# yzqin/s4g-release

Hardware: AMD Instinct MI355X
Metric: scenes/sec (25.6k-pt clouds) end-to-end grasp inference (higher is better)
Workload: dtype f32 (f16x2 split)

## Files before the change

### s4g_release_amd/csrc/fps.hip

```cpp
#include <stdlib.h>
#include <string.h>


#include "s4g_common.h"

namespace s4g {

constexpr int FPS_THREADS = 1024;
constexpr int FPS_TIE_PAR = 5;
constexpr int FPS_MAX_WAVES = 16;
constexpr uint32_t FPS_JMASK = 0x7FFFFFu;

typedef float fps_v2f __attribute__((ext_vector_type(2)));

struct FpsSlot {
  uint32_t d;
  uint32_t tie;
  float x, y, z;
  uint32_t d2;
  uint32_t key2;
  uint32_t pad;
};

struct FpsExtra {
// ... 144 lines not shown
        wkey = min(wkey, dpp_u32<0x141>(wkey));
        const bool was_hit = v != s.d;
        uint32_t kb = (was_hit && s.d2 == bnd) ? slots[ej].key2 : 0xFFFFFFFFu;
        kb = min(kb, dpp_u32<0xB1>(kb));
        kb = min(kb, dpp_u32<0x4E>(kb));
        kb = min(kb, dpp_u32<0x141>(kb));
        if (!((uint32_t)__builtin_amdgcn_readlane(wkey, 0) < (uint32_t)__builtin_amdgcn_readlane(kb, 0))) break;
      }
      take(k);
    }
  }
  cur = (int)((uint32_t)__builtin_amdgcn_readlane(s.tie, xl) & FPS_JMASK);
  cx = __uint_as_float(__builtin_amdgcn_readlane(__float_as_uint(s.x), xl));
  cy = __uint_as_float(__builtin_amdgcn_readlane(__float_as_uint(s.y), xl));
  cz = __uint_as_float(__builtin_amdgcn_readlane(__float_as_uint(s.z), xl));
  fx = __uint_as_float(__builtin_amdgcn_readlane(__float_as_uint(s.x), xl0));
  fy = __uint_as_float(__builtin_amdgcn_readlane(__float_as_uint(s.y), xl0));
  fz = __uint_as_float(__builtin_amdgcn_readlane(__float_as_uint(s.z), xl0));
  if (wave == 0 && lane < np) {
    const FpsSlot e = slots[(pw >> (4 * lane)) & 15u];
    out_i[lane] = (IdxT)(e.tie & FPS_JMASK);
    if (cout_i) {
      cout_i[lane] = e.x;
      cout_i[M + lane] = e.y;
      cout_i[2 * M + lane] = e.z;
    }
    if (dout_i) dout_i[lane] = __uint_as_float(my_d);
  }
  picked_waves = pw;
  return np;
}

template <int PPT, int LO, int HI>
__device__ __forceinline__ void fps_pick(const float (&x)[PPT],
                                         const float (&y)[PPT],
                                         const float (&z)[PPT], int pw, int wl,
                                         float& sx, float& sy, float& sz) {
  if constexpr (HI - LO == 1) {
    sx = __uint_as_float(__builtin_amdgcn_readlane(__float_as_uint(x[LO]), wl));
    sy = __uint_as_float(__builtin_amdgcn_readlane(__float_as_uint(y[LO]), wl));
    sz = __uint_as_float(__builtin_amdgcn_readlane(__float_as_uint(z[LO]), wl));
  } else {
    constexpr int MID = (LO + HI) / 2;
    if (pw < MID)
      fps_pick<PPT, LO, MID>(x, y, z, pw, wl, sx, sy, sz);
    else
      fps_pick<PPT, MID, HI>(x, y, z, pw, wl, sx, sy, sz);
  }
}

template <int THREADS, int PPT, bool FMAD, typename IdxT>
__global__ __launch_bounds__(THREADS) void fps_reg_kernel(
    const float* __restrict__ xyz, int N, int M, IdxT* __restrict__ idx,
    float* __restrict__ ctr, int lg_bs, int M_run, float* __restrict__ md_out, FpsExtra ex) {
  constexpr int WAVES = THREADS / 64;
  __shared__ FpsSlot slots[2][FPS_MAX_WAVES];
  const int b = blockIdx.x;
  const int t = threadIdx.x;
  const int lane = t & 63;
  const int wave = t >> 6;
  const float* __restrict__ px = xyz + (size_t)b * 3 * N;
  const float* __restrict__ py = px + N;
  const float* __restrict__ pz = py + N;
  IdxT* __restrict__ out = idx + (size_t)b * M;
  float* __restrict__ cout = ctr ? ctr + (size_t)b * 3 * M : nullptr;
  float* __restrict__ dout = ex.dist ? ex.dist + (size_t)b * M : nullptr;
  if (ex.run && ex.run[b] == 0) {
    for (int i = t; i < M_run; i += THREADS) {
      out[i] = (IdxT)i;
      if (cout) {
        cout[i] = px[i];
        cout[M + i] = py[i];
        cout[2 * M + i] = pz[i];
      }
    }
    return;
  }

  float x[PPT], y[PPT], z[PPT], md[PPT];
#pragma unroll
  for (int p = 0; p < PPT; ++p) {
    const int j = t + THREADS * p;
    const bool ok = j < N;
    const int jj = ok ? j : 0;
    x[p] = px[jj];
    y[p] = py[jj];
    z[p] = pz[jj];
    md[p] = ok ? __builtin_inff() : -1.0f;
  }
  const uint32_t bs_mask = (1u << lg_bs) - 1u;
  const uint32_t rkey = (__brev((uint32_t)t & bs_mask) >> (32 - lg_bs)) << 23;

  int cur = 0;
  float cx = px[0], cy = py[0], cz = pz[0];
  if (t == 0) {
    out[0] = 0;
    if (cout) {
      cout[0] = cx;
      cout[M] = cy;
      cout[2 * M] = cz;
    }
    if (dout) dout[0] = __builtin_inff();
  }

  for (int i = 1; i < M_run; ++i) {
    float best = 0.0f;
    int bestp = -1;
    const fps_v2f cx2 = {cx, cx}, cy2 = {cy, cy}, cz2 = {cz, cz};
#pragma unroll
    for (int p = 0; p + 1 < PPT; p += 2) {
      const fps_v2f xv = {x[p], x[p + 1]}, yv = {y[p], y[p + 1]}, zv = {z[p], z[p + 1]};
      const fps_v2f dx = xv - cx2, dy = yv - cy2, dz = zv - cz2;
      fps_v2f d;
      if constexpr (FMAD) {
        d = __builtin_elementwise_fma(dz, dz, __builtin_elementwise_fma(dy, dy, dx * dx));
      } else {
        d = (dx * dx + dy * dy) + dz * dz;
      }
#pragma unroll
      for (int e = 0; e < 2; ++e) {
        float m;
        asm("v_min_f32 %0, %1, %2" : "=v"(m) : "v"(d[e]), "v"(md[p + e]));
        md[p + e] = m;
        if (m > best) {
          best = m;
          bestp = p + e;
        }
      }
    }
    if constexpr (PPT & 1) {
      constexpr int p = PPT - 1;
      const float d = dist2<FMAD>(cx, cy, cz, x[p], y[p], z[p]);
      float m;
      asm("v_min_f32 %0, %1, %2" : "=v"(m) : "v"(d), "v"(md[p]));
      md[p] = m;
      if (m > best) {
        best = m;
        bestp = p;
      }
    }
    const uint32_t jbest =
        (bestp < 0) ? (uint32_t)cur : (uint32_t)(t + THREADS * bestp);
    const uint32_t tie = rkey | jbest;
    const uint32_t dbits = __float_as_uint(best);
    const uint32_t wmax = wave_max_u32(dbits);
    uint64_t win = __ballot(dbits == wmax);
    uint32_t wtie;
    if (__popcll(win) > 1) {
      wtie = wave_min_u32((dbits == wmax) ? tie : 0xFFFFFFFFu);
      win = __ballot(dbits == wmax && tie == wtie);
    } else {
      wtie = __builtin_amdgcn_readlane(tie, __ffsll((unsigned long long)win) - 1);
    }
    const int wl = __ffsll((unsigned long long)win) - 1;
    const int pw = __builtin_amdgcn_readlane(bestp, wl);
    float sx = cx, sy = cy, sz = cz;
    if (pw >= 0) fps_pick<PPT, 0, PPT>(x, y, z, pw, wl, sx, sy, sz);
    uint32_t dwin;
    fps_block_exchange<WAVES>(slots[i & 1], wave, lane, wmax, wtie, sx, sy, sz, cur,
                       cx, cy, cz, &dwin);
    if (t == 0) {
      out[i] = (IdxT)cur;
      if (cout) {
        cout[i] = cx;
        cout[M + i] = cy;
        cout[2 * M + i] = cz;
      }
      if (dout) dout[i] = __uint_as_float(dwin);
    }
  }
  if (md_out) {
#pragma unroll
    for (int p = 0; p < PPT; ++p) {
      const int j = t + THREADS * p;
      if (j < N) md_out[(size_t)b * N + j] = md[p];
    }
  }
}

template <bool FMAD, typename IdxT>
__global__ __launch_bounds__(FPS_THREADS) void fps_stream_kernel(
    const float* __restrict__ xyz, int N, int M, IdxT* __restrict__ idx,
    float* __restrict__ ctr, float* __restrict__ temp, int lg_bs) {
  __shared__ FpsSlot slots[2][FPS_MAX_WAVES];
  const int b = blockIdx.x;
  const int t = threadIdx.x;
  const int lane = t & 63;
  const int wave = t >> 6;
  const float* __restrict__ px = xyz + (size_t)b * 3 * N;
  const float* __restrict__ py = px + N;
  const float* __restrict__ pz = py + N;
  float* __restrict__ md = temp + (size_t)b * N;
  IdxT* __restrict__ out = idx + (size_t)b * M;
  float* __restrict__ cout = ctr ? ctr + (size_t)b * 3 * M : nullptr;

  for (int j = t; j < N; j += FPS_THREADS) md[j] = __builtin_inff();
  const uint32_t bs_mask = (1u << lg_bs) - 1u;
  const uint32_t rkey = (__brev((uint32_t)t & bs_mask) >> (32 - lg_bs)) << 23;

  int cur = 0;
  float cx = px[0], cy = py[0], cz = pz[0];
  if (t == 0) {
    out[0] = 0;
    if (cout) {
      cout[0] = cx;
      cout[M] = cy;
      cout[2 * M] = cz;
    }
  }

  for (int i = 1; i < M; ++i) {
    float best = 0.0f;
    int bestj = -1;
    for (int j = t; j < N; j += FPS_THREADS) {
      const float d = dist2<FMAD>(cx, cy, cz, px[j], py[j], pz[j]);
      const float o = md[j];
      const float m = (d < o) ? d : o;
      if (d < o) md[j] = m;
      if (m > best) {
        best = m;
        bestj = j;
      }
    }
    const uint32_t jbest = (bestj < 0) ? (uint32_t)cur : (uint32_t)bestj;
    const uint32_t tie = rkey | jbest;
    const uint32_t dbits = __float_as_uint(best);
    const uint32_t wmax = wave_max_u32(dbits);
    const uint32_t wtie = wave_min_u32((dbits == wmax) ? tie : 0xFFFFFFFFu);
// ... 361 lines not shown
      for (int u = 0; u < AU; ++u) {
        const int sp = sp0 + u * FPS_SORT_THREADS;
        j[u] = sp < N ? __hip_atomic_load(&pm[sp], __ATOMIC_RELAXED, __HIP_MEMORY_SCOPE_AGENT) : 0;
      }
      float c[AU][3];
#pragma unroll
      for (int u = 0; u < AU; ++u)
#pragma unroll
        for (int a = 0; a < 3; ++a) c[u][a] = p[(size_t)a * N + j[u]];
#pragma unroll
      for (int u = 0; u < AU; ++u) {
        const int sp = sp0 + u * FPS_SORT_THREADS;
        if (sp < aos_cap) out[sp] = make_float4(c[u][0], c[u][1], c[u][2], __int_as_float(j[u]));
      }
    }
  }
}

__device__ __forceinline__ float fps_max3(float a, float b, float c) {
  float r;
  asm("v_max3_f32 %0, %1, %2, %3" : "=v"(r) : "v"(a), "v"(b), "v"(c));
  return r;
}

template <int PPT, int LO, int HI>
__device__ __forceinline__ float fps_pick_md(const float (&md)[PPT], int pw) {
  if constexpr (HI - LO == 1) {
    float v = md[LO];
    asm volatile("; fps pick %1" : "+v"(v) : "n"(LO));
    return v;
  } else {
    constexpr int MID = (LO + HI) / 2;
    if (pw < MID) return fps_pick_md<PPT, LO, MID>(md, pw);
    return fps_pick_md<PPT, MID, HI>(md, pw);
  }
}

template <int PPT, int LO, int HI>
__device__ __forceinline__ void fps_pick_slot(const float (&x)[PPT], const float (&y)[PPT],
                                              const float (&z)[PPT], const float (&md)[PPT], int pw,
                                              float& vx, float& vy, float& vz, float& vm) {
  if constexpr (HI - LO == 1) {
    vx = x[LO];
    vy = y[LO];
    vz = z[LO];
    vm = md[LO];
    asm volatile("; fps pick" : "+v"(vx), "+v"(vy), "+v"(vz), "+v"(vm));
  } else {
    constexpr int MID = (LO + HI) / 2;
    if (pw < MID)
      fps_pick_slot<PPT, LO, MID>(x, y, z, md, pw, vx, vy, vz, vm);
    else
      fps_pick_slot<PPT, MID, HI>(x, y, z, md, pw, vx, vy, vz, vm);
  }
}

template <int PPT, int LO, int HI, bool FMAD>
__device__ __forceinline__ void fps_update_slot(const float (&x)[PPT], const float (&y)[PPT],
                                                const float (&z)[PPT], float (&md)[PPT], int p,
                                                float cx, float cy, float cz, float& gmax) {
  if constexpr (HI - LO == 1) {
    float xl = x[LO];
    asm volatile("; fps slot %1" : "+v"(xl) : "n"(LO));
    const float d = dist2<FMAD>(cx, cy, cz, xl, y[LO], z[LO]);
    float m;
    asm volatile("v_min_f32 %0, %1, %2" : "=v"(m) : "v"(d), "v"(md[LO]));
    md[LO] = m;
    const uint32_t g = wave_max_u32(__float_as_uint(m));
    gmax = __uint_as_float(g);
  } else {
    constexpr int MID = (LO + HI) / 2;
    if (p < MID)
      fps_update_slot<PPT, LO, MID, FMAD>(x, y, z, md, p, cx, cy, cz, gmax);
    else
      fps_update_slot<PPT, MID, HI, FMAD>(x, y, z, md, p, cx, cy, cz, gmax);
  }
}

template <int THREADS, int PPT, bool FMAD, typename IdxT, int MAXP>
__global__ __launch_bounds__(THREADS) void fps_pruned_kernel(const float* __restrict__ xyz,
                                                             const int* __restrict__ perm,
                                                             const float* __restrict__ gbox,
                                                             const float* __restrict__ md_in, int i0,
                                                             int N, int M, IdxT* __restrict__ idx,
                                                             float* __restrict__ ctr, int lg_bs,
                                                             float* __restrict__ dist) {
  constexpr int WAVES = THREADS / 64;
  constexpr int GPL = (PPT + 63) / 64;
  constexpr bool SPEC = MAXP > 1;
  __shared__ FpsSlot slots[2][FPS_MAX_WAVES];
  extern __shared__ uint16_t orig[];
  const int b = blockIdx.x;
  const int t = threadIdx.x;
  const int lane = t & 63;
  const int wave = t >> 6;
  const float* __restrict__ px = xyz + (size_t)b * 3 * N;
  const float* __restrict__ py = px + N;
  const float* __restrict__ pz = py + N;
  const int* __restrict__ pb = perm + (size_t)b * N;
  IdxT* __restrict__ out = idx + (size_t)b * M;
  float* __restrict__ cout = ctr ? ctr + (size_t)b * 3 * M : nullptr;
  float* __restrict__ dout = dist ? dist + (size_t)b * M : nullptr;
  const uint32_t bs_mask = (1u << lg_bs) - 1u;
  auto tie_key = [&](uint32_t j) { return ((__brev(j & bs_mask) >> (32 - lg_bs)) << 23) | j; };

  float x[PPT], y[PPT], z[PPT], md[PPT];
// ... 61 lines not shown
  if constexpr (SPEC) {
    if (t == 0) {
      FpsSlot s0;
      s0.d = s0.tie = s0.d2 = s0.key2 = s0.pad = 0u;
      s0.x = cx;
      s0.y = cy;
      s0.z = cz;
      slots[1][0] = s0;
    }
    __syncthreads();
  }
  S4G_FPS_ACC_DECL();
  for (int i = i0; i < M;) {
    uint32_t wmax, wtie, wd2 = 0u, wkey2 = 0u;
    float sx = cx, sy = cy, sz = cz;
    [[maybe_unused]] const unsigned long long st0 = S4G_FPS_T();
    uint32_t gbits[GPL];
#pragma unroll 1
    for (int q = 0; q < npend; ++q) {
    float ux = cx, uy = cy, uz = cz;
    if constexpr (SPEC) {
      const FpsSlot& e = slots[xpar ^ 1][(pwaves >> (4 * q)) & 15u];
      ux = e.x;
      uy = e.y;
      uz = e.z;
    }
#pragma unroll
    for (int r = 0; r < GPL; ++r) {
      const bool live = 64 * r + lane < PPT;
      const float tx = fps_max3(__fsub_rn(blx[r], ux), __fsub_rn(ux, bhx[r]), 0.f);
      const float ty = fps_max3(__fsub_rn(bly[r], uy), __fsub_rn(uy, bhy[r]), 0.f);
      const float tz = fps_max3(__fsub_rn(blz[r], uz), __fsub_rn(uz, bhz[r]), 0.f);
      float lb;
      if constexpr (FMAD) {
        lb = __fmaf_rn(tz, tz, __fmaf_rn(ty, ty, __fmul_rn(tx, tx)));
      } else {
        lb = __fadd_rn(__fadd_rn(__fmul_rn(tx, tx), __fmul_rn(ty, ty)), __fmul_rn(tz, tz));
      }
      const uint64_t need = __ballot(live && lb < mg[r]);
      S4G_FPS_ACC(5, __popcll(need));
      if (need) {
#pragma unroll
        for (int p8 = 0; p8 < 64 && 64 * r + p8 < PPT; p8 += 8) {
          if (__builtin_expect(((need >> p8) & 0xFFull) != 0ull, 0)) {
#pragma unroll
            for (int e = 0; e < 8; ++e) {
              constexpr int dummy = 0;
              (void)dummy;
              const int p = 64 * r + p8 + e;
              if (p < PPT) {
                if ((need >> (p8 + e)) & 1ull) {
                  float xl = x[p];
                  asm volatile("; fps slot" : "+v"(xl));
                  const float d = dist2<FMAD>(ux, uy, uz, xl, y[p], z[p]);
                  float m;
                  const float old = md[p];
                  asm volatile("v_min_f32 %0, %1, %2" : "=v"(m) : "v"(d), "v"(old));
                  md[p] = m;
                  const uint32_t gm = __builtin_amdgcn_readlane(__float_as_uint(mg[r]), p8 + e);
                  if (__ballot(__float_as_uint(old) == gm && m < old)) {
                    const uint32_t g = wave_max_u32(__float_as_uint(m));
                    if (lane == p8 + e) mg[r] = __uint_as_float(g);
                  }
                }
              }
            }
          }
        }
      }
      gbits[r] = live ? __float_as_uint(mg[r]) : 0u;
    }
    }
    [[maybe_unused]] const unsigned long long st1 = S4G_FPS_T();
    uint32_t lmax = gbits[0];
#pragma unroll
    for (int r = 1; r < GPL; ++r) lmax = max(lmax, gbits[r]);
    wmax = wave_max_u32(lmax);
    if (wmax == 0u) {
      wtie = wave_min_u32(rkey | (uint32_t)cur);
    } else {
      uint32_t best_key = 0xFFFFFFFFu, second_key = 0xFFFFFFFFu;
      int nbest = 0;
      bool tie_par = false;
      if constexpr (GPL == 1) {
        const uint64_t gtie = __ballot(gbits[0] == wmax);
        tie_par = __popcll(gtie) > FPS_TIE_PAR;
        if (__builtin_expect(tie_par, 0)) {
          float* __restrict__ mdl = reinterpret_cast<float*>(orig + THREADS * PPT) + t;
#pragma unroll
          for (int pp = 0; pp < PPT; ++pp)
            if ((gtie >> pp) & 1ull) mdl[pp * THREADS] = md[pp];
          uint32_t kl = 0xFFFFFFFFu, k2l = 0xFFFFFFFFu;
          int pl = 0;
          uint64_t gleft = gtie;
#pragma unroll 1
          while (gleft) {
            const int pp = __builtin_amdgcn_readfirstlane(__ffsll((unsigned long long)gleft) - 1);
            gleft &= gleft - 1;
            const int s = 64 * (WAVES * pp + wave) + lane;
            const uint32_t kk = tie_key(orig[s < N ? s : 0]);
            const bool hit = s < N && __float_as_uint(mdl[pp * THREADS]) == wmax;
            if (hit && kk < kl) {
              k2l = kl;
              kl = kk;
              pl = pp;
            } else if (hit && kk < k2l) {
              k2l = kk;
// ... 331 lines not shown
  auto take = [&](size_t bytes) {
    char* r = p ? p + off : nullptr;
    off += (bytes + 255) & ~(size_t)255;
    return r;
  };
  const int64_t l2_groups = 8 * (int64_t)fps_l2_slots(N);
  const int64_t gbox_groups = (N + 63) / 64 + 256 > l2_groups ? (N + 63) / 64 + 256 : l2_groups;
  w.gbox = (float*)take(sizeof(float) * 6 * B * gbox_groups);
  w.val_out = (int*)take(sizeof(int) * n);
  w.aos = N > (int64_t)512 * 50 ? (float4*)take(sizeof(float4) * (size_t)B * 512 * fps_l2_slots(N)) : nullptr;
  w.total = off;
  return w;
}

static bool fps_use_pruned_l2(int64_t N, int64_t M) {
  if (N <= (int64_t)512 * 50 || N > FPS_L2_CAP_BIG || M < 64) return false;
  const char* e = s4g::knob("S4G_FPS_MODE");
  return !(e && e[0] == 'd');
}

static bool fps_use_pruned(int64_t N, int64_t M) {
  const char* e = s4g::knob("S4G_FPS_MODE");
  if (e && e[0] == 'd') return false;
  if (N > (int64_t)512 * 50) return false;
  if (e && e[0] == 'p') return N > 512 * 5;
  return N > 512 * 20 || (N > 512 * 10 && (M < 0 || M >= 2048));
}

static int ref_block_lg(int64_t n) {
  int cnt = 0;
  int64_t x = n - 1;
  while (x > 0) {
    x >>= 1;
    ++cnt;
  }
  if (cnt > 9) cnt = 9;
  if (cnt < 4) cnt = 4;
  return cnt;
}

template <bool FMAD>
__global__ __launch_bounds__(256) void fps_prefix_check_kernel(const float* __restrict__ ctr,
                                                               const float* __restrict__ dist, int M1,
                                                               int M2, int* __restrict__ run) {
  __shared__ float4 step[256];
  const int b = blockIdx.y;
  const int j = blockIdx.x * 256 + threadIdx.x;
  const float* __restrict__ cx = ctr + (size_t)b * 3 * M1;
  const float* __restrict__ cy = cx + M1;
  const float* __restrict__ cz = cy + M1;
  const float* __restrict__ D = dist + (size_t)b * M1;
  const int jj = j < M1 ? j : 0;
  const float sx = cx[jj], sy = cy[jj], sz = cz[jj];
  float m = __builtin_inff();
  bool bad = false;
  for (int k0 = 0; k0 + 1 < M2; k0 += 256) {
    const int kk = k0 + threadIdx.x;
    __syncthreads();
    if (kk + 1 < M2) step[threadIdx.x] = make_float4(cx[kk], cy[kk], cz[kk], D[kk + 1]);
    __syncthreads();
    const int n = min(256, M2 - 1 - k0);
#pragma unroll 4
    for (int q = 0; q < n; ++q) {
      const float4 c = step[q];
      const float d = dist2<FMAD>(c.x, c.y, c.z, sx, sy, sz);
      m = d < m ? d : m;
      const int k = k0 + q;
      bad |= !(c.w > 0.f) || !(c.w < __builtin_inff()) || (j > k + 1 && j < M1 && !(m < c.w)) ||
             (j == k + 1 && __float_as_uint(m) != __float_as_uint(c.w));
    }
  }
  if (__syncthreads_or(bad) && threadIdx.x == 0) atomicOr(&run[b], 1);
}

static int launch_fps_cell_sort(const float* xyz, int64_t B, int64_t N, int G, int* perm, float* gbox,
                                float4* aos, int aos_cap, hipStream_t stream) {
  constexpr size_t lds = sizeof(uint32_t) * (FPS_SORT_WORDS + 3 * 256 + 64 * 64 / 2 + 7 * (FPS_SORT_THREADS / 64) + 8);
  static LdsAttrCache lds_cache;
  if (int rc = allow_dynamic_lds(reinterpret_cast<const void*>(&fps_cell_sort_kernel), lds, lds_cache)) return rc;
  hipLaunchKernelGGL(fps_cell_sort_kernel, dim3((unsigned)B), dim3(FPS_SORT_THREADS), lds, stream, xyz, (int)N, G,
                     perm, gbox, aos, aos_cap);
  S4G_LAUNCH_CHECK();
  return S4G_OK;
}

template <bool FMAD, typename IdxT>
static int launch_fps(const float* xyz, int64_t B, int64_t N, int64_t M,
                      IdxT* idx, float* ctr, void* ws, size_t ws_bytes,
                      hipStream_t stream, FpsExtra ex = FpsExtra{nullptr, nullptr}) {
  const int lg = ref_block_lg(N);
  const dim3 grid((unsigned)B);

  if (fps_use_pruned(N, M) && M > FPS_PRUNED_MIN_PICKS && B < (1 << 16)) {
    const FpsSortWs w = fps_sort_ws(ws, B, N);
    if (ws && ws_bytes >= w.total) {
      const int G = 8 * (N <= 512 * 10 ? 10 : N <= 512 * 20 ? 20 : N <= 512 * 32 ? 32 : 50);
      if (int rc = launch_fps_cell_sort(xyz, B, N, G, w.val_out, w.gbox, nullptr, 0, stream)) return rc;
#define S4G_FPS_PRUNED_LAUNCH(T, P, S)                                                             \
  {                                                                                                \
    static LdsAttrCache lds_cache;                                                                 \
    if (int rc = allow_dynamic_lds(reinterpret_cast<const void*>(&fps_pruned_kernel<T, P, FMAD, IdxT, S>), lds, lds_cache)) return rc;  \
    hipLaunchKernelGGL((fps_pruned_kernel<T, P, FMAD, IdxT, S>), grid, dim3(T), lds, stream, xyz,  \
                       w.val_out, w.gbox, (const float*)nullptr, 1, (int)N, (int)M, idx, ctr, lg,  \
                       ex.dist);                                                                   \
  }
#define S4G_FPS_PRUNED(T, P)                                                                       \
  if (N <= (int64_t)T * P) {                                                                       \
    const size_t lds = (sizeof(uint16_t) + sizeof(float)) * T * P;    \
    S4G_FPS_PRUNED_LAUNCH(T, P, 4)                                                                 \
    S4G_LAUNCH_CHECK();                                                                            \
    return S4G_OK;                                                                                 \
  }
      S4G_FPS_PRUNED(512, 10)
      S4G_FPS_PRUNED(512, 20)
      S4G_FPS_PRUNED(512, 32)
      S4G_FPS_PRUNED(512, 50)
#undef S4G_FPS_PRUNED
#undef S4G_FPS_PRUNED_LAUNCH
    }
  }

  bool launched = false;
#define S4G_FPS_CASE(T, P)                                                   \
  if (!launched && N <= (int64_t)T * P) {                                    \
    hipLaunchKernelGGL((fps_reg_kernel<T, P, FMAD, IdxT>), grid, dim3(T), 0, \
                       stream, xyz, (int)N, (int)M, idx, ctr, lg, (int)M,    \
                       (float*)nullptr, ex);                                 \
    S4G_LAUNCH_CHECK();                                                      \
    launched = true;                                                         \
  }
  S4G_FPS_CASE(256, 1)
  S4G_FPS_CASE(512, 1)
  S4G_FPS_CASE(512, 2)
  S4G_FPS_CASE(512, 5)
  S4G_FPS_CASE(512, 10)
  S4G_FPS_CASE(512, 20)
  S4G_FPS_CASE(512, 32)
  S4G_FPS_CASE(512, 50)
#undef S4G_FPS_CASE
  if (launched) return S4G_OK;
  if (fps_use_pruned_l2(N, M) && B < (1 << 16)) {
    const FpsSortWs w2 = fps_sort_ws(ws, B, N);
    if (ws && ws_bytes >= w2.total) {
      const int slots = fps_l2_slots(N);
      if (int rc = launch_fps_cell_sort(xyz, B, N, 8 * slots, w2.val_out, w2.gbox, w2.aos, 512 * slots, stream)) return rc;
      if (slots == 100)
        hipLaunchKernelGGL((fps_pruned_l2_kernel<512, 100, FMAD, IdxT, 2>), grid, dim3(512), 0, stream, xyz,
                           w2.aos, w2.gbox, (int)N, (int)M, idx, ctr, lg, ex.dist);
      else
        hipLaunchKernelGGL((fps_pruned_l2_kernel<512, 128, FMAD, IdxT, 2>), grid, dim3(512), 0, stream, xyz,
                           w2.aos, w2.gbox, (int)N, (int)M, idx, ctr, lg, ex.dist);
      S4G_LAUNCH_CHECK();
      return S4G_OK;
    }
  }
  if (ex.dist) return S4G_EUNSUPPORTED;
  if (ws_bytes < (size_t)B * (size_t)N * sizeof(float) || ws == nullptr)
    return S4G_EWORKSPACE;
  hipLaunchKernelGGL((fps_stream_kernel<FMAD, IdxT>), grid, dim3(FPS_THREADS), 0, stream,
                     xyz, (int)N, (int)M, idx, ctr, (float*)ws, lg);
  S4G_LAUNCH_CHECK();
  return S4G_OK;
}

size_t fps_workspace_bytes(int64_t B, int64_t N) {
  if (N <= 0 || B <= 0) return 0;
  if (N <= (int64_t)512 * 50) return fps_use_pruned(N, -1) ? fps_sort_ws(nullptr, B, N).total : 0;
  if (N <= FPS_L2_CAP_BIG) return fps_sort_ws(nullptr, B, N).total;
  return (size_t)B * (size_t)N * sizeof(float);
}

}

#ifdef S4G_FPS_STAMPS
extern "C" int s4g_debug_fps_stamps(unsigned long long* host_out_64x8x8, int reset) {
  hipError_t e = hipMemcpyFromSymbol(host_out_64x8x8, HIP_SYMBOL(s4g::g_fps_acc), sizeof(unsigned long long) * 64 * 8 * 8);
  if (e == hipSuccess && reset) {
    static unsigned long long zeros[64 * 8 * 8];
    e = hipMemcpyToSymbol(HIP_SYMBOL(s4g::g_fps_acc), zeros, sizeof(zeros));
  }
// ... 71 lines not shown
```

### s4g_release_amd/csrc/three_nn.hip

```cpp
#include "grid.h"

#include <stdlib.h>

namespace s4g {

constexpr int NN_THREADS = 256;

__device__ __forceinline__ int nn_safe_index(int j, int N2) { return (unsigned)j < (unsigned)N2 ? j : 0; }

template <bool FMAD, bool WEIGHTS, typename IdxT>
__global__ __launch_bounds__(NN_THREADS) void three_nn_kernel(
    const float* __restrict__ q, const float* __restrict__ key, int N1, int N2,
    float eps, IdxT* __restrict__ idx, float* __restrict__ d2out) {
  const int b = blockIdx.y;
  const int i = blockIdx.x * NN_THREADS + threadIdx.x;
  const float* __restrict__ qx = q + (size_t)b * 3 * N1;
  const float* __restrict__ kx = key + (size_t)b * 3 * N2;
  const float* __restrict__ ky = kx + N2;
  const float* __restrict__ kz = ky + N2;
  const int ii = i < N1 ? i : N1 - 1;
  const float x1 = qx[ii], y1 = qx[N1 + ii], z1 = qx[2 * N1 + ii];

  float b0 = __builtin_inff(), b1 = 0.0f, b2 = 0.0f;
  int i0 = -1, i1 = 0, i2 = 0;
// ... 170 lines not shown
          if (a1 < a0) { const float q = a0; a0 = a1; a1 = q; }
        }
      }
    }
    float kth = 0.f;
    for (int r = 0; r < 4; ++r) {
      const float m = __uint_as_float(wave_min_u32(__float_as_uint(a0)));
      kth = m;
      const uint64_t own = __ballot(a0 == m);
      if (lane == (int)(__ffsll((unsigned long long)own) - 1)) {
        a0 = a1;
        a1 = a2;
        a2 = a3;
        a3 = __builtin_inff();
      }
    }
    if (lane == 0) {
      __hip_atomic_store(d3s + s, kth, __ATOMIC_RELAXED, __HIP_MEMORY_SCOPE_AGENT);
      __threadfence();
    }
  }
  int last = 0;
  if (lane == 0) last = atomicAdd(hdr + 8, 1) == NN_SAMPLES - 1;
  last = __builtin_amdgcn_readfirstlane(last);
  if (!last) return;
  __threadfence();
  {
    const float d = __hip_atomic_load(d3s + lane, __ATOMIC_RELAXED, __HIP_MEMORY_SCOPE_AGENT);
    const bool ok = d > 0.f && d < __builtin_inff();
    const int n = __popcll(__ballot(ok));
    int rank = 0;
    for (int q = 0; q < NN_SAMPLES; ++q) {
      const float dq = __uint_as_float(__builtin_amdgcn_readlane(__float_as_uint(d), q));
      const bool okq = dq > 0.f && dq < __builtin_inff();
      rank += (okq && (dq < d || (dq == d && q < lane))) ? 1 : 0;
    }
    const uint64_t mid = __ballot(ok && rank == n / 2);
    float cell = 0.f;
    if (mid) cell = factor * sqrtf(__uint_as_float(__builtin_amdgcn_readlane(__float_as_uint(d), (int)(__ffsll((unsigned long long)mid) - 1))));
    if (lane == 0) {
      if (!(cell > 0.f) || !(cell < 1e18f)) {
        out[0] = 1.0f;
        out[1] = -1.0f;
      } else {
        const float edge = cell * (1.0f - 1e-3f);
        out[0] = 1.0f / cell;
        out[1] = edge * edge;
      }
    }
  }
}

template <bool FMAD, bool WEIGHTS, typename IdxT>
__global__ __launch_bounds__(NN_THREADS) void three_nn_grid_kernel(
    const float* __restrict__ key, int N1, int N2, float inv_h, float d2_done, GridWs ws,
    CellWs cw, float eps, IdxT* __restrict__ idx, float* __restrict__ out,
    int* __restrict__ fail_list, int* __restrict__ fail_count,
    const float* __restrict__ cell_dev = nullptr) {
  if (cell_dev) {
    inv_h = cell_dev[0];
    d2_done = cell_dev[1];
  }
  const int b = blockIdx.y;
  int r = blockIdx.x * NN_THREADS + threadIdx.x;
  if (r >= N1) return;
  const int* __restrict__ cnt = cw.ncell + ((size_t)gridDim.y + b) * GR_RANGES;
  int g = 0;
#pragma unroll
  for (int k = 0; k < GR_RANGES - 1; ++k) {
    const int c = cnt[k];
    if (g == k && r >= c) {
      r -= c;
      g = k + 1;
    }
  }
  const float4 qr = cw.sorted[((size_t)b * GR_RANGES + g) * N1 + r];
  const int i = __float_as_int(qr.w);
  const float x1 = qr.x, y1 = qr.y, z1 = qr.z;
  const float* __restrict__ kx = key + (size_t)b * 3 * N2;
  const float ox = kx[0], oy = kx[N2], oz = kx[2 * N2];
  const bool exact = ws.flags[b] == 0 && grid_coord_ok(x1, ox, inv_h) &&
                     grid_coord_ok(y1, oy, inv_h) && grid_coord_ok(z1, oz, inv_h);
  float b0 = __builtin_inff(), b1 = __builtin_inff(), b2 = __builtin_inff();
  int i0 = 0x7FFFFFFF, i1 = 0x7FFFFFFF, i2 = 0x7FFFFFFF;
  if (exact) {
    const int icx = grid_coord(x1, ox, inv_h), icy = grid_coord(y1, oy, inv_h),
              icz = grid_coord(z1, oz, inv_h);
    const __amdgpu_buffer_rsrc_t rrec = __builtin_amdgcn_make_buffer_rsrc(
        (void*)(ws.sorted + (size_t)b * GR_RANGES * N2), 0, GR_RANGES * N2 * 16, 0x00020000);
    const int* __restrict__ starts_b = ws.starts + (size_t)b * GR_RANGES * GR_START_STRIDE;
    const int x0 = (icx - 1) & 31;
    const bool wrap = x0 > GR_DIM - 3;
    const int xe = wrap ? GR_DIM : x0 + 3;
    int beg[9], n0[9], beg1[9], n1[9];
#pragma unroll
    for (int rr = 0; rr < 9; ++rr) {
      const int zz = (icz + rr / 3 - 1) & 31, yy = (icy + rr % 3 - 1) & 31;
      const int* __restrict__ st = starts_b + grid_range(yy, zz) * GR_START_STRIDE +
                                   grid_local_row(yy, zz);
      beg[rr] = st[x0];
      n0[rr] = st[xe] - beg[rr];
      beg1[rr] = 0;
      n1[rr] = 0;
    }
    if (__ballot(wrap) != 0ull) {
#pragma unroll
      for (int rr = 0; rr < 9; ++rr) {
        const int zz = (icz + rr / 3 - 1) & 31, yy = (icy + rr % 3 - 1) & 31;
        const int* __restrict__ st = starts_b + grid_range(yy, zz) * GR_START_STRIDE +
                                     grid_local_row(yy, zz);
        beg1[rr] = st[0];
        n1[rr] = wrap ? st[(x0 + 3) & 31] - beg1[rr] : 0;
      }
    }
    auto visit = [&](const float4 p, bool valid) {
      const int j = valid ? __float_as_int(p.w) : 0x7FFFFFFF;
      float d = dist2<FMAD>(p.x, p.y, p.z, x1, y1, z1);
      d = valid ? d : __builtin_inff();
      const bool c0 = nn_less(d, j, b0, i0), c1 = nn_less(d, j, b1, i1), c2 = nn_less(d, j, b2, i2);
      const bool c01 = c0 | c1;
      b2 = c01 ? b1 : (c2 ? d : b2);
      i2 = c01 ? i1 : (c2 ? j : i2);
      b1 = c0 ? b0 : (c1 ? d : b1);
      i1 = c0 ? i0 : (c1 ? j : i1);
      b0 = c0 ? d : b0;
      i0 = c0 ? j : i0;
    };
    auto rec_off = [&](int rr, int t) -> int {
      const int j = t < n0[rr] ? beg[rr] + t : beg1[rr] + (t - n0[rr]);
      return t < n0[rr] + n1[rr] ? j * 16 : 0x7FFFFFF0;
    };
#pragma unroll
    for (int grp = 0; grp < 3; ++grp) {
      float4 p[12];
#pragma unroll
      for (int u = 0; u < 12; ++u)
        p[u] = __builtin_bit_cast(float4, __builtin_amdgcn_raw_buffer_load_b128(
                                              rrec, rec_off(grp * 3 + u / 4, u % 4), 0, 0));
#pragma unroll
      for (int u = 0; u < 12; ++u)
        asm volatile("" : "+v"(p[u].x), "+v"(p[u].y), "+v"(p[u].z), "+v"(p[u].w));
#pragma unroll
      for (int u = 0; u < 12; ++u) {
        const int rr = grp * 3 + u / 4;
        visit(p[u], (u % 4) < n0[rr] + n1[rr]);
      }
#pragma unroll
      for (int k = 0; k < 3; ++k) {
        const int rr = grp * 3 + k;
        const int n = n0[rr] + n1[rr];
        for (int t = 4; t < n; t += 4) {
          float4 q4[4];
#pragma unroll
          for (int u = 0; u < 4; ++u)
            q4[u] = __builtin_bit_cast(float4, __builtin_amdgcn_raw_buffer_load_b128(
                                                   rrec, rec_off(rr, t + u), 0, 0));
#pragma unroll
          for (int u = 0; u < 4; ++u)
            asm volatile("" : "+v"(q4[u].x), "+v"(q4[u].y), "+v"(q4[u].z), "+v"(q4[u].w));
#pragma unroll
          for (int u = 0; u < 4; ++u) visit(q4[u], t + u < n);
        }
      }
    }
  }
  const bool done = exact && i2 != 0x7FFFFFFF && b2 < d2_done;
  if (done) {
    nn_write<WEIGHTS, IdxT>(idx, out, ((size_t)b * N1 + i) * 3, i0, i1, i2, b0, b1, b2, eps, N2);
  } else {
    fail_list[atomicAdd(fail_count, 1)] = b * N1 + i;
  }
}

template <bool FMAD, bool WEIGHTS, typename IdxT>
__global__ __launch_bounds__(NN_THREADS) void three_nn_fallback_kernel(
    const float* __restrict__ q, const float* __restrict__ key, int N1, int N2, float eps,
    IdxT* __restrict__ idx, float* __restrict__ out, const int* __restrict__ fail_list,
    const int* __restrict__ fail_count) {
  constexpr int NW = NN_THREADS / 64;
  __shared__ float sd[NW * 3];
  __shared__ int sj[NW * 3];
  const int lane = threadIdx.x & 63, wave = threadIdx.x >> 6;
  const int count = *fail_count;
  auto insert = [](float d, int j, float& b0, float& b1, float& b2, int& i0, int& i1, int& i2) {
    const bool c0 = nn_less(d, j, b0, i0), c1 = nn_less(d, j, b1, i1), c2 = nn_less(d, j, b2, i2);
    const bool c01 = c0 | c1;
    b2 = c01 ? b1 : (c2 ? d : b2);
    i2 = c01 ? i1 : (c2 ? j : i2);
    b1 = c0 ? b0 : (c1 ? d : b1);
    i1 = c0 ? i0 : (c1 ? j : i1);
    b0 = c0 ? d : b0;
    i0 = c0 ? j : i0;
  };
  auto merge3 = [&](float& b0, float& b1, float& b2, int& i0, int& i1, int& i2, float* rd, int* rj) {
#pragma unroll
    for (int k = 0; k < 3; ++k) {
      const uint32_t dm = wave_min_u32(__float_as_uint(b0));
      const uint32_t jm = wave_min_u32(__float_as_uint(b0) == dm ? (uint32_t)i0 : 0xFFFFFFFFu);
      rd[k] = __uint_as_float(dm);
      rj[k] = (int)jm;
      if (__float_as_uint(b0) == dm && (uint32_t)i0 == jm) {
        b0 = b1; i0 = i1; b1 = b2; i1 = i2; b2 = __builtin_inff(); i2 = 0x7FFFFFFF;
      }
    }
  };
  for (int f = blockIdx.x; f < count; f += gridDim.x) {
    const int qi = fail_list[f];
    const int b = qi / N1, i = qi - b * N1;
    const float* __restrict__ qx = q + (size_t)b * 3 * N1;
    const float* __restrict__ kx = key + (size_t)b * 3 * N2;
    const float x1 = qx[i], y1 = qx[N1 + i], z1 = qx[2 * N1 + i];
    float b0 = __builtin_inff(), b1 = __builtin_inff(), b2 = __builtin_inff();
    int i0 = 0x7FFFFFFF, i1 = 0x7FFFFFFF, i2 = 0x7FFFFFFF;
    constexpr int FU = 8;
    for (int j0 = threadIdx.x; j0 < N2; j0 += NN_THREADS * FU) {
      float px[FU], py[FU], pz[FU];
#pragma unroll
      for (int u = 0; u < FU; ++u) {
        const int j = j0 + NN_THREADS * u < N2 ? j0 + NN_THREADS * u : 0;
        px[u] = kx[j];
        py[u] = kx[N2 + j];
        pz[u] = kx[2 * N2 + j];
      }
#pragma unroll
      for (int u = 0; u < FU; ++u) {
        const bool valid = j0 + NN_THREADS * u < N2;
        const float d = dist2<FMAD>(px[u], py[u], pz[u], x1, y1, z1);
        insert(valid ? d : __builtin_inff(), valid ? j0 + NN_THREADS * u : 0x7FFFFFFF, b0, b1, b2,
               i0, i1, i2);
      }
    }
    float rd[3];
    int rj[3];
    merge3(b0, b1, b2, i0, i1, i2, rd, rj);
    if (lane == 0) {
#pragma unroll
      for (int k = 0; k < 3; ++k) {
        sd[wave * 3 + k] = rd[k];
        sj[wave * 3 + k] = rj[k];
      }
    }
    __syncthreads();
    if (wave == 0) {
      b0 = lane < NW * 3 ? sd[lane] : __builtin_inff();
      i0 = lane < NW * 3 ? sj[lane] : 0x7FFFFFFF;
      b1 = b2 = __builtin_inff();
      i1 = i2 = 0x7FFFFFFF;
      merge3(b0, b1, b2, i0, i1, i2, rd, rj);
      if (lane == 0)
        nn_write<WEIGHTS, IdxT>(idx, out, ((size_t)b * N1 + i) * 3, rj[0], rj[1], rj[2], rd[0],
                                rd[1], rd[2], eps, N2);
    }
    __syncthreads();
  }
}

__global__ __launch_bounds__(NN_THREADS) void interp_weights_kernel(
    const float* __restrict__ d2, int64_t n, float eps, float* __restrict__ w) {
  const int64_t t = (int64_t)blockIdx.x * NN_THREADS + threadIdx.x;
  if (t >= n) return;
  const float a = d2[t * 3 + 0], b = d2[t * 3 + 1], c = d2[t * 3 + 2];
  const float ia = __fdiv_rn(1.0f, a < eps ? eps : a);
  const float ib = __fdiv_rn(1.0f, b < eps ? eps : b);
  const float ic = __fdiv_rn(1.0f, c < eps ? eps : c);
  const float s = __fadd_rn(__fadd_rn(ia, ib), ic);
  w[t * 3 + 0] = __fdiv_rn(ia, s);
  w[t * 3 + 1] = __fdiv_rn(ib, s);
  w[t * 3 + 2] = __fdiv_rn(ic, s);
}

}

extern "C" int s4g_three_nn_f32(const float* q_b3n1, const float* k_b3n2,
                                int64_t B, int64_t N1, int64_t N2,
                                int64_t* idx_bn3, float* d2_bn3, void* ws,
                                size_t ws_bytes, int flags,
                                s4g_stream_t stream) {
  (void)ws;
  (void)ws_bytes;
  if (B < 0 || N1 < 0 || N2 < 3 || B > 65535 || N2 >= (1ll << 31) ||
      N1 >= (1ll << 31))
    return S4G_EINVAL;
  if (B == 0 || N1 == 0) return S4G_OK;
  if (!q_b3n1 || !k_b3n2 || !idx_bn3 || !d2_bn3) return S4G_EINVAL;
  hipStream_t st = (hipStream_t)stream;
  if (flags & S4G_FLAG_FMAD)
    return s4g::launch_three_nn_scan<true, false, int64_t>(q_b3n1, k_b3n2, B, N1, N2, 0.f, idx_bn3, d2_bn3, st);
  return s4g::launch_three_nn_scan<false, false, int64_t>(q_b3n1, k_b3n2, B, N1, N2, 0.f, idx_bn3, d2_bn3, st);
}

extern "C" int s4g_three_nn_weights_i32(const float* q_b3n1, const float* k_b3n2,
                                        int64_t B, int64_t N1, int64_t N2,
                                        float eps, int32_t* idx_bn3,
                                        float* w_bn3, void* ws, size_t ws_bytes,
                                        int flags, s4g_stream_t stream) {
  (void)ws;
  (void)ws_bytes;
  if (B < 0 || N1 < 0 || N2 < 3 || B > 65535 || N2 >= (1ll << 31) ||
      N1 >= (1ll << 31))
    return S4G_EINVAL;
  if (B == 0 || N1 == 0) return S4G_OK;
  if (!q_b3n1 || !k_b3n2 || !idx_bn3 || !w_bn3) return S4G_EINVAL;
  hipStream_t st = (hipStream_t)stream;
  if (flags & S4G_FLAG_FMAD)
    return s4g::launch_three_nn_scan<true, true, int32_t>(q_b3n1, k_b3n2, B, N1, N2, eps, idx_bn3, w_bn3, st);
  return s4g::launch_three_nn_scan<false, true, int32_t>(q_b3n1, k_b3n2, B, N1, N2, eps, idx_bn3, w_bn3, st);
// ... 1 lines not shown

static size_t nn_fail_bytes(int64_t B, int64_t N1) {
  return (sizeof(int) * ((size_t)B * N1 + s4g::NN_HDR_WORDS) + 63) & ~(size_t)63;
}

extern "C" size_t s4g_three_nn_grid_workspace_bytes(int64_t B, int64_t N1, int64_t N2) {
  return s4g::grid_ws_bytes(B, N2) + nn_fail_bytes(B, N1) + s4g::cell_ws_bytes(B, N1);
}

extern "C" size_t s4g_three_nn_grid_header_offset(int64_t B, int64_t N2) { return s4g::grid_ws_bytes(B, N2); }

namespace s4g {

template <bool WEIGHTS, typename IdxT>
static int launch_three_nn_grid(const float* q, const float* k, int64_t B, int64_t N1, int64_t N2,
                                float eps, float cell, IdxT* idx, float* out, void* ws,
                                size_t ws_bytes, int flags, hipStream_t st) {
  const bool auto_cell = cell < 0.f;
  if (B < 0 || N1 < 0 || N2 < 3 || B > 65535 || N2 > GR_MAX_POINTS || N1 >= (1ll << 31) ||
      B * N1 >= (1ll << 31) || (!auto_cell && (!(cell > 0.f) || !(cell < 1e18f))))
    return S4G_EINVAL;
  if (B == 0 || N1 == 0) return S4G_OK;
  if (!q || !k || !idx || !out || !ws) return S4G_EINVAL;
  if (ws_bytes < s4g_three_nn_grid_workspace_bytes(B, N1, N2)) return S4G_EWORKSPACE;
  const GridWs g = grid_ws_carve(ws, B, N2);
  int* fail_count = reinterpret_cast<int*>((char*)ws + grid_ws_bytes(B, N2));
  int* fail_list = fail_count + NN_HDR_WORDS;
  const CellWs cw = cell_ws_carve((char*)fail_count + nn_fail_bytes(B, N1), B, N1);
  hipError_t e = hipMemsetAsync(fail_count, 0, sizeof(int) * 16, st);
  if (e != hipSuccess) return (int)e;
  float* cell_dev = nullptr;
  if (auto_cell) {
    cell_dev = reinterpret_cast<float*>(fail_count + 4);
    constexpr float factor = 1.75f;
    hipLaunchKernelGGL(nn_auto_cell_kernel, dim3(NN_SAMPLES), dim3(64), 0, st, k, (int)B, (int)N2, fail_count, factor);
    S4G_LAUNCH_CHECK();
    cell = 1.0f;
  }
  const float inv_h = 1.0f / cell;
  if (int rc = launch_grid_build_queries(k, q, B, N2, N1, inv_h, g, cw, st, false, cell_dev)) return rc;
  const float edge = cell * (1.0f - 1e-3f);
  const float d2_done = edge * edge;
  const dim3 grid((unsigned)((N1 + NN_THREADS - 1) / NN_THREADS), (unsigned)B);
  const bool fmad = (flags & S4G_FLAG_FMAD) != 0;
  if (fmad)
    hipLaunchKernelGGL((three_nn_grid_kernel<true, WEIGHTS, IdxT>), grid, dim3(NN_THREADS), 0, st,
                       k, (int)N1, (int)N2, inv_h, d2_done, g, cw, eps, idx, out, fail_list,
                       fail_count, (const float*)cell_dev);
  else
    hipLaunchKernelGGL((three_nn_grid_kernel<false, WEIGHTS, IdxT>), grid, dim3(NN_THREADS), 0, st,
                       k, (int)N1, (int)N2, inv_h, d2_done, g, cw, eps, idx, out, fail_list,
                       fail_count, (const float*)cell_dev);
  S4G_LAUNCH_CHECK();
  if (fmad)
    hipLaunchKernelGGL((three_nn_fallback_kernel<true, WEIGHTS, IdxT>), dim3(512), dim3(NN_THREADS),
                       0, st, q, k, (int)N1, (int)N2, eps, idx, out, fail_list, fail_count);
  else
    hipLaunchKernelGGL((three_nn_fallback_kernel<false, WEIGHTS, IdxT>), dim3(512), dim3(NN_THREADS),
                       0, st, q, k, (int)N1, (int)N2, eps, idx, out, fail_list, fail_count);
  S4G_LAUNCH_CHECK();
  return S4G_OK;
}

}

extern "C" int s4g_three_nn_weights_grid_i32(const float* q_b3n1, const float* k_b3n2,
                                             int64_t B, int64_t N1, int64_t N2, float eps,
                                             float cell, int32_t* idx_bn3, float* w_bn3,
                                             void* ws, size_t ws_bytes, int flags,
                                             s4g_stream_t stream) {
  return s4g::launch_three_nn_grid<true, int32_t>(q_b3n1, k_b3n2, B, N1, N2, eps, cell, idx_bn3,
                                                  w_bn3, ws, ws_bytes, flags, (hipStream_t)stream);
}

extern "C" int s4g_three_nn_grid_f32(const float* q_b3n1, const float* k_b3n2, int64_t B,
                                     int64_t N1, int64_t N2, float cell, int64_t* idx_bn3,
                                     float* d2_bn3, void* ws, size_t ws_bytes, int flags,
                                     s4g_stream_t stream) {
  return s4g::launch_three_nn_grid<false, int64_t>(q_b3n1, k_b3n2, B, N1, N2, 0.f, cell, idx_bn3,
                                                   d2_bn3, ws, ws_bytes, flags, (hipStream_t)stream);
}

extern "C" int s4g_interp_weights_f32(const float* d2_bn3, int64_t B,
                                      int64_t N1, float eps, float* w_bn3,
                                      s4g_stream_t stream) {
  if (B < 0 || N1 < 0) return S4G_EINVAL;
  const int64_t n = B * N1;
  if (n == 0) return S4G_OK;
  if (!d2_bn3 || !w_bn3) return S4G_EINVAL;
  const dim3 grid((unsigned)((n + s4g::NN_THREADS - 1) / s4g::NN_THREADS));
  hipLaunchKernelGGL(s4g::interp_weights_kernel, grid, dim3(s4g::NN_THREADS), 0,
                     (hipStream_t)stream, d2_bn3, n, eps, w_bn3);
  S4G_LAUNCH_CHECK();
  return S4G_OK;
}
```

Baseline: 2035.

## Fuse three-NN fallback into grid kernel and simplify FPS verify and reg kernel

The separate three_nn fallback launch is removed. Each grid-kernel workgroup now queues its own failed queries in shared memory and brute-force scans them in-block, which saves a kernel launch at the cost of more serialized work in blocks with failures. The FPS verify kernel gains a fast path for blocks beyond M2 and moves the checks on D values and on the exact-match case out of the inner loop. The unused M_run and md_out parameters are dropped from fps_reg_kernel, and an unpacked distance helper replaces dist2 in one slot-update path.

```diff
diff --git a/s4g_release_amd/csrc/fps.hip b/s4g_release_amd/csrc/fps.hip
--- a/s4g_release_amd/csrc/fps.hip
+++ b/s4g_release_amd/csrc/fps.hip
@@ -220,7 +220,7 @@
 template <int THREADS, int PPT, bool FMAD, typename IdxT>
 __global__ __launch_bounds__(THREADS) void fps_reg_kernel(
     const float* __restrict__ xyz, int N, int M, IdxT* __restrict__ idx,
-    float* __restrict__ ctr, int lg_bs, int M_run, float* __restrict__ md_out, FpsExtra ex) {
+    float* __restrict__ ctr, int lg_bs, FpsExtra ex) {
   constexpr int WAVES = THREADS / 64;
   __shared__ FpsSlot slots[2][FPS_MAX_WAVES];
   const int b = blockIdx.x;
@@ -234,7 +234,7 @@
   float* __restrict__ cout = ctr ? ctr + (size_t)b * 3 * M : nullptr;
   float* __restrict__ dout = ex.dist ? ex.dist + (size_t)b * M : nullptr;
   if (ex.run && ex.run[b] == 0) {
-    for (int i = t; i < M_run; i += THREADS) {
+    for (int i = t; i < M; i += THREADS) {
       out[i] = (IdxT)i;
       if (cout) {
         cout[i] = px[i];
@@ -271,7 +271,7 @@
     if (dout) dout[0] = __builtin_inff();
   }
 
-  for (int i = 1; i < M_run; ++i) {
+  for (int i = 1; i < M; ++i) {
     float best = 0.0f;
     int bestp = -1;
     const fps_v2f cx2 = {cx, cx}, cy2 = {cy, cy}, cz2 = {cz, cz};
@@ -335,13 +335,6 @@
         cout[2 * M + i] = cz;
       }
       if (dout) dout[i] = __uint_as_float(dwin);
-    }
-  }
-  if (md_out) {
-#pragma unroll
-    for (int p = 0; p < PPT; ++p) {
-      const int j = t + THREADS * p;
-      if (j < N) md_out[(size_t)b * N + j] = md[p];
     }
   }
 }
@@ -809,6 +802,19 @@
       fps_pick_slot<PPT, LO, MID>(x, y, z, md, pw, vx, vy, vz, vm);
     else
       fps_pick_slot<PPT, MID, HI>(x, y, z, md, pw, vx, vy, vz, vm);
+  }
+}
+
+template <bool FMAD>
+__device__ __forceinline__ float fps_dist2_unpacked(float cx, float cy, float cz, float x, float y, float z) {
+  float dx, dy, dz;
+  asm("v_sub_f32 %0, %1, %2" : "=v"(dx) : "v"(x), "v"(cx));
+  asm("v_sub_f32 %0, %1, %2" : "=v"(dy) : "v"(y), "v"(cy));
+  asm("v_sub_f32 %0, %1, %2" : "=v"(dz) : "v"(z), "v"(cz));
+  if constexpr (FMAD) {
+    return __fmaf_rn(dz, dz, __fmaf_rn(dy, dy, __fmul_rn(dx, dx)));
+  } else {
+    return __fadd_rn(__fadd_rn(__fmul_rn(dx, dx), __fmul_rn(dy, dy)), __fmul_rn(dz, dz));
   }
 }
 
@@ -976,7 +982,7 @@
                 if ((need >> (p8 + e)) & 1ull) {
                   float xl = x[p];
                   asm volatile("; fps slot" : "+v"(xl));
-                  const float d = dist2<FMAD>(ux, uy, uz, xl, y[p], z[p]);
+                  const float d = fps_dist2_unpacked<FMAD>(ux, uy, uz, xl, y[p], z[p]);
                   float m;
                   const float old = md[p];
                   asm volatile("v_min_f32 %0, %1, %2" : "=v"(m) : "v"(d), "v"(old));
@@ -1414,25 +1420,44 @@
   const float* __restrict__ D = dist + (size_t)b * M1;
   const int jj = j < M1 ? j : 0;
   const float sx = cx[jj], sy = cy[jj], sz = cz[jj];
+  const bool behind = (int)(blockIdx.x * 256) >= M2;
   float m = __builtin_inff();
+  float mj = 0.f;
   bool bad = false;
+  bool bad_d = false;
   for (int k0 = 0; k0 + 1 < M2; k0 += 256) {
     const int kk = k0 + threadIdx.x;
     __syncthreads();
-    if (kk + 1 < M2) step[threadIdx.x] = make_float4(cx[kk], cy[kk], cz[kk], D[kk + 1]);
+    if (kk + 1 < M2) {
+      const float dn = D[kk + 1];
+      step[threadIdx.x] = make_float4(cx[kk], cy[kk], cz[kk], dn);
+      bad_d |= !(dn > 0.f) || !(dn < __builtin_inff());
+    }
     __syncthreads();
     const int n = min(256, M2 - 1 - k0);
+    if (behind) {
 #pragma unroll 4
-    for (int q = 0; q < n; ++q) {
-      const float4 c = step[q];
-      const float d = dist2<FMAD>(c.x, c.y, c.z, sx, sy, sz);
-      m = d < m ? d : m;
-      const int k = k0 + q;
-      bad |= !(c.w > 0.f) || !(c.w < __builtin_inff()) || (j > k + 1 && j < M1 && !(m < c.w)) ||
-             (j == k + 1 && __float_as_uint(m) != __float_as_uint(c.w));
-    }
-  }
-  if (__syncthreads_or(bad) && threadIdx.x == 0) atomicOr(&run[b], 1);
+      for (int q = 0; q < n; ++q) {
+        const float4 c = step[q];
+        const float d = dist2<FMAD>(c.x, c.y, c.z, sx, sy, sz);
+        m = d < m ? d : m;
+        bad |= !(m < c.w);
+      }
+    } else {
+#pragma unroll 4
+      for (int q = 0; q < n; ++q) {
+        const float4 c = step[q];
+        const float d = dist2<FMAD>(c.x, c.y, c.z, sx, sy, sz);
+        m = d < m ? d : m;
+        const int k = k0 + q;
+        mj = j == k + 1 ? m : mj;
+        bad |= j > k + 1 && !(m < c.w);
+      }
+    }
+  }
+  if (j >= M1) bad = false;
+  if (j >= 1 && j < M2) bad |= __float_as_uint(mj) != __float_as_uint(D[j]);
+  if (__syncthreads_or(bad || bad_d) && threadIdx.x == 0) atomicOr(&run[b], 1);
 }
 
 static int launch_fps_cell_sort(const float* xyz, int64_t B, int64_t N, int G, int* perm, float* gbox,
@@ -1486,8 +1511,7 @@
 #define S4G_FPS_CASE(T, P)                                                   \
   if (!launched && N <= (int64_t)T * P) {                                    \
     hipLaunchKernelGGL((fps_reg_kernel<T, P, FMAD, IdxT>), grid, dim3(T), 0, \
-                       stream, xyz, (int)N, (int)M, idx, ctr, lg, (int)M,    \
-                       (float*)nullptr, ex);                                 \
+                       stream, xyz, (int)N, (int)M, idx, ctr, lg, ex);       \
     S4G_LAUNCH_CHECK();                                                      \
     launched = true;                                                         \
   }
diff --git a/s4g_release_amd/csrc/three_nn.hip b/s4g_release_amd/csrc/three_nn.hip
--- a/s4g_release_amd/csrc/three_nn.hip
+++ b/s4g_release_amd/csrc/three_nn.hip
@@ -246,6 +246,76 @@
 }
 
 template <bool FMAD, bool WEIGHTS, typename IdxT>
+__device__ __forceinline__ void nn_scan_query(const float* __restrict__ kx, int N2, float x1, float y1, float z1,
+                                              float eps, IdxT* __restrict__ idx, float* __restrict__ out, size_t o,
+                                              float* __restrict__ sd, int* __restrict__ sj) {
+  constexpr int NW = NN_THREADS / 64;
+  const int lane = threadIdx.x & 63, wave = threadIdx.x >> 6;
+  auto insert = [](float d, int j, float& b0, float& b1, float& b2, int& i0, int& i1, int& i2) {
+    const bool c0 = nn_less(d, j, b0, i0), c1 = nn_less(d, j, b1, i1), c2 = nn_less(d, j, b2, i2);
+    const bool c01 = c0 | c1;
+    b2 = c01 ? b1 : (c2 ? d : b2);
+    i2 = c01 ? i1 : (c2 ? j : i2);
+    b1 = c0 ? b0 : (c1 ? d : b1);
+    i1 = c0 ? i0 : (c1 ? j : i1);
+    b0 = c0 ? d : b0;
+    i0 = c0 ? j : i0;
+  };
+  auto merge3 = [&](float& b0, float& b1, float& b2, int& i0, int& i1, int& i2, float* rd, int* rj) {
+#pragma unroll
+    for (int k = 0; k < 3; ++k) {
+      const uint32_t dm = wave_min_u32(__float_as_uint(b0));
+      const uint32_t jm = wave_min_u32(__float_as_uint(b0) == dm ? (uint32_t)i0 : 0xFFFFFFFFu);
+      rd[k] = __uint_as_float(dm);
+      rj[k] = (int)jm;
+      if (__float_as_uint(b0) == dm && (uint32_t)i0 == jm) {
+        b0 = b1; i0 = i1; b1 = b2; i1 = i2; b2 = __builtin_inff(); i2 = 0x7FFFFFFF;
+      }
+    }
+  };
+  float b0 = __builtin_inff(), b1 = __builtin_inff(), b2 = __builtin_inff();
+  int i0 = 0x7FFFFFFF, i1 = 0x7FFFFFFF, i2 = 0x7FFFFFFF;
+  constexpr int FU = 8;
+  for (int j0 = threadIdx.x; j0 < N2; j0 += NN_THREADS * FU) {
+    float px[FU], py[FU], pz[FU];
+#pragma unroll
+    for (int u = 0; u < FU; ++u) {
+      const int j = j0 + NN_THREADS * u < N2 ? j0 + NN_THREADS * u : 0;
+      px[u] = kx[j];
+      py[u] = kx[N2 + j];
+      pz[u] = kx[2 * N2 + j];
+    }
+#pragma unroll
+    for (int u = 0; u < FU; ++u) {
+      const bool valid = j0 + NN_THREADS * u < N2;
+      const float d = dist2<FMAD>(px[u], py[u], pz[u], x1, y1, z1);
+      insert(valid ? d : __builtin_inff(), valid ? j0 + NN_THREADS * u : 0x7FFFFFFF, b0, b1, b2,
+             i0, i1, i2);
+    }
+  }
+  float rd[3];
+  int rj[3];
+  merge3(b0, b1, b2, i0, i1, i2, rd, rj);
+  if (lane == 0) {
+#pragma unroll
+    for (int k = 0; k < 3; ++k) {
+      sd[wave * 3 + k] = rd[k];
+      sj[wave * 3 + k] = rj[k];
+    }
+  }
+  __syncthreads();
+  if (wave == 0) {
+    b0 = lane < NW * 3 ? sd[lane] : __builtin_inff();
+    i0 = lane < NW * 3 ? sj[lane] : 0x7FFFFFFF;
+    b1 = b2 = __builtin_inff();
+    i1 = i2 = 0x7FFFFFFF;
+    merge3(b0, b1, b2, i0, i1, i2, rd, rj);
+    if (lane == 0) nn_write<WEIGHTS, IdxT>(idx, out, o, rj[0], rj[1], rj[2], rd[0], rd[1], rd[2], eps, N2);
+  }
+  __syncthreads();
+}
+
+template <bool FMAD, bool WEIGHTS, typename IdxT>
 __global__ __launch_bounds__(NN_THREADS) void three_nn_grid_kernel(
     const float* __restrict__ key, int N1, int N2, float inv_h, float d2_done, GridWs ws,
     CellWs cw, float eps, IdxT* __restrict__ idx, float* __restrict__ out,
@@ -255,9 +325,16 @@
     inv_h = cell_dev[0];
     d2_done = cell_dev[1];
   }
+  __shared__ float4 wg_fail[NN_THREADS];
+  __shared__ int wg_nfail;
+  __shared__ float sd[NN_THREADS / 64 * 3];
+  __shared__ int sj[NN_THREADS / 64 * 3];
   const int b = blockIdx.y;
   int r = blockIdx.x * NN_THREADS + threadIdx.x;
-  if (r >= N1) return;
+  const float* __restrict__ kx = key + (size_t)b * 3 * N2;
+  if (threadIdx.x == 0) wg_nfail = 0;
+  __syncthreads();
+  if (r < N1) {
   const int* __restrict__ cnt = cw.ncell + ((size_t)gridDim.y + b) * GR_RANGES;
   int g = 0;
 #pragma unroll
@@ -271,7 +348,6 @@
   const float4 qr = cw.sorted[((size_t)b * GR_RANGES + g) * N1 + r];
   const int i = __float_as_int(qr.w);
   const float x1 = qr.x, y1 = qr.y, z1 = qr.z;
-  const float* __restrict__ kx = key + (size_t)b * 3 * N2;
   const float ox = kx[0], oy = kx[N2], oz = kx[2 * N2];
   const bool exact = ws.flags[b] == 0 && grid_coord_ok(x1, ox, inv_h) &&
                      grid_coord_ok(y1, oy, inv_h) && grid_coord_ok(z1, oz, inv_h);
@@ -363,89 +439,15 @@
     nn_write<WEIGHTS, IdxT>(idx, out, ((size_t)b * N1 + i) * 3, i0, i1, i2, b0, b1, b2, eps, N2);
   } else {
     fail_list[atomicAdd(fail_count, 1)] = b * N1 + i;
-  }
-}
-
-template <bool FMAD, bool WEIGHTS, typename IdxT>
-__global__ __launch_bounds__(NN_THREADS) void three_nn_fallback_kernel(
-    const float* __restrict__ q, const float* __restrict__ key, int N1, int N2, float eps,
-    IdxT* __restrict__ idx, float* __restrict__ out, const int* __restrict__ fail_list,
-    const int* __restrict__ fail_count) {
-  constexpr int NW = NN_THREADS / 64;
-  __shared__ float sd[NW * 3];
-  __shared__ int sj[NW * 3];
-  const int lane = threadIdx.x & 63, wave = threadIdx.x >> 6;
-  const int count = *fail_count;
-  auto insert = [](float d, int j, float& b0, float& b1, float& b2, int& i0, int& i1, int& i2) {
-    const bool c0 = nn_less(d, j, b0, i0), c1 = nn_less(d, j, b1, i1), c2 = nn_less(d, j, b2, i2);
-    const bool c01 = c0 | c1;
-    b2 = c01 ? b1 : (c2 ? d : b2);
-    i2 = c01 ? i1 : (c2 ? j : i2);
-    b1 = c0 ? b0 : (c1 ? d : b1);
-    i1 = c0 ? i0 : (c1 ? j : i1);
-    b0 = c0 ? d : b0;
-    i0 = c0 ? j : i0;
-  };
-  auto merge3 = [&](float& b0, float& b1, float& b2, int& i0, int& i1, int& i2, float* rd, int* rj) {
-#pragma unroll
-    for (int k = 0; k < 3; ++k) {
-      const uint32_t dm = wave_min_u32(__float_as_uint(b0));
-      const uint32_t jm = wave_min_u32(__float_as_uint(b0) == dm ? (uint32_t)i0 : 0xFFFFFFFFu);
-      rd[k] = __uint_as_float(dm);
-      rj[k] = (int)jm;
-      if (__float_as_uint(b0) == dm && (uint32_t)i0 == jm) {
-        b0 = b1; i0 = i1; b1 = b2; i1 = i2; b2 = __builtin_inff(); i2 = 0x7FFFFFFF;
-      }
-    }
-  };
-  for (int f = blockIdx.x; f < count; f += gridDim.x) {
-    const int qi = fail_list[f];
-    const int b = qi / N1, i = qi - b * N1;
-    const float* __restrict__ qx = q + (size_t)b * 3 * N1;
-    const float* __restrict__ kx = key + (size_t)b * 3 * N2;
-    const float x1 = qx[i], y1 = qx[N1 + i], z1 = qx[2 * N1 + i];
-    float b0 = __builtin_inff(), b1 = __builtin_inff(), b2 = __builtin_inff();
-    int i0 = 0x7FFFFFFF, i1 = 0x7FFFFFFF, i2 = 0x7FFFFFFF;
-    constexpr int FU = 8;
-    for (int j0 = threadIdx.x; j0 < N2; j0 += NN_THREADS * FU) {
-      float px[FU], py[FU], pz[FU];
-#pragma unroll
-      for (int u = 0; u < FU; ++u) {
-        const int j = j0 + NN_THREADS * u < N2 ? j0 + NN_THREADS * u : 0;
-        px[u] = kx[j];
-        py[u] = kx[N2 + j];
-        pz[u] = kx[2 * N2 + j];
-      }
-#pragma unroll
-      for (int u = 0; u < FU; ++u) {
-        const bool valid = j0 + NN_THREADS * u < N2;
-        const float d = dist2<FMAD>(px[u], py[u], pz[u], x1, y1, z1);
-        insert(valid ? d : __builtin_inff(), valid ? j0 + NN_THREADS * u : 0x7FFFFFFF, b0, b1, b2,
-               i0, i1, i2);
-      }
-    }
-    float rd[3];
-    int rj[3];
-    merge3(b0, b1, b2, i0, i1, i2, rd, rj);
-    if (lane == 0) {
-#pragma unroll
-      for (int k = 0; k < 3; ++k) {
-        sd[wave * 3 + k] = rd[k];
-        sj[wave * 3 + k] = rj[k];
-      }
-    }
-    __syncthreads();
-    if (wave == 0) {
-      b0 = lane < NW * 3 ? sd[lane] : __builtin_inff();
-      i0 = lane < NW * 3 ? sj[lane] : 0x7FFFFFFF;
-      b1 = b2 = __builtin_inff();
-      i1 = i2 = 0x7FFFFFFF;
-      merge3(b0, b1, b2, i0, i1, i2, rd, rj);
-      if (lane == 0)
-        nn_write<WEIGHTS, IdxT>(idx, out, ((size_t)b * N1 + i) * 3, rj[0], rj[1], rj[2], rd[0],
-                                rd[1], rd[2], eps, N2);
-    }
-    __syncthreads();
+    wg_fail[atomicAdd(&wg_nfail, 1)] = make_float4(x1, y1, z1, __int_as_float(i));
+  }
+  }
+  __syncthreads();
+  const int nfail = wg_nfail;
+  for (int f = 0; f < nfail; ++f) {
+    const float4 qf = wg_fail[f];
+    nn_scan_query<FMAD, WEIGHTS, IdxT>(kx, N2, qf.x, qf.y, qf.z, eps, idx, out,
+                                       ((size_t)b * N1 + __float_as_int(qf.w)) * 3, sd, sj);
   }
 }
 
@@ -553,13 +555,6 @@
                        k, (int)N1, (int)N2, inv_h, d2_done, g, cw, eps, idx, out, fail_list,
                        fail_count, (const float*)cell_dev);
   S4G_LAUNCH_CHECK();
-  if (fmad)
-    hipLaunchKernelGGL((three_nn_fallback_kernel<true, WEIGHTS, IdxT>), dim3(512), dim3(NN_THREADS),
-                       0, st, q, k, (int)N1, (int)N2, eps, idx, out, fail_list, fail_count);
-  else
-    hipLaunchKernelGGL((three_nn_fallback_kernel<false, WEIGHTS, IdxT>), dim3(512), dim3(NN_THREADS),
-                       0, st, q, k, (int)N1, (int)N2, eps, idx, out, fail_list, fail_count);
-  S4G_LAUNCH_CHECK();
   return S4G_OK;
 }
 
```

After: 2024. About the same (-0.5%).
